# kirilllzaitsev/vision_mtl

Measured on AMD Instinct MI355X. Metric: images/sec fwd+bwd, basic model 128x256, higher is better.
Workload: dtype f32

## Files before the change

### include/vmtl.h

```cpp
#ifndef VMTL_H
#define VMTL_H

#ifdef __cplusplus
extern "C" {
#endif

#define VMTL_ACT_NONE 0
#define VMTL_ACT_RELU 1
#define VMTL_ACT_HSWISH 2
#define VMTL_ACT_HSIGMOID 3
#define VMTL_ACT_SIGMOID 4

#define VMTL_PREC_FP32 0
#define VMTL_PREC_BF16 1

const char* vmtl_version(void);
const char* vmtl_last_error_string(void);
int vmtl_reload_env(void);
int vmtl_timestamp(long long* out, void* stream);


int vmtl_conv2d_fwd(const float* x, const float* wp, const float* bias, float* y, float* stats,
                    int B, int H, int W, int Cs, int Ho, int Wo, int ldy, int Nw, int Cout,
                    int KH, int KW, int stride, int pad, int act, int shuffle, void* stream);
// ... 3 lines not shown
int vmtl_conv2d_ksplit(int B, int Ho, int Wo, int ldy, int Ktot);
int vmtl_conv2d_fwd_ws(const float* x, const float* wp, const float* bias, float* y, float* ws, int B, int H, int W, int Cs,
                       int Ho, int Wo, int ldy, int Nw, int Cout, int KH, int KW, int stride, int pad, void* stream);
int vmtl_conv2d_fwd_ws_p(const float* x, const float* wp, const float* bias, float* y, float* ws, int B, int H, int W,
                         int Cs, int Ho, int Wo, int ldy, int Nw, int Cout, int KH, int KW, int stride, int pad,
                         int precision, void* stream);
int vmtl_conv2d_stats_rows(int B, int Ho, int Wo, int ldy);
int vmtl_conv2d_stats_block(int B, int Ho, int Wo, int ldy);

int vmtl_conv1x1_stats_block(int M, int ldy, int Ks, int variant);
int vmtl_conv1x1_stats_rows(int M, int ldy, int Ks, int variant);
int vmtl_conv1x1_fwd(const float* x, const float* wp, const float* bias, float* y, float* stats, int M, int Ks, int ldy,
                     int Nw, int Cout, void* stream);
int vmtl_conv1x1_cat_fwd(const float* x, int K1, const float* x2, int K2s, const float* wp, const float* bias, float* y,
                         float* stats, int M, int ldy, int Nw, int Cout, void* stream);
int vmtl_conv1x1_cat_dgrad(const float* dy, const float* wp, float* dx, int N1, float* dx2, int N2s, int N2, int M,
                           int Ks, void* stream);
int vmtl_conv1x1_cat_wgrad(const float* x, int K1, const float* x2, int K2s, const float* dy, float* slabs, int splits,
                           int M, int ldy, int Nw, void* stream);
int vmtl_conv1x1_cat_wgrad_p(const float* x, int K1, const float* x2, int K2s, const float* dy, float* slabs, int splits,
                             int M, int ldy, int Nw, int precision, void* stream);
int vmtl_conv1x1_bn_fwd(const float* x, const float* coef_a, const float* coef_c, int act_in, float* a_out,
                        const float* wp, const float* bias, float* y, float* stats, int M, int Ks, int ldy, int Nw,
                        int Cout, void* stream);
int vmtl_conv1x1_bnbwd(const float* dy, const float* wp, float* dz, float* stats, const float* ez_x,
                       const float* ez_mean, const float* ez_invstd, const float* ez_gamma, const float* ez_beta,
                       int ez_act, int M, int Ks, int ldy, int Nw, int Cout, void* stream);
int vmtl_conv1x1_bn_res_fwd(const float* x, const float* coef_a, const float* coef_c, int act_in, const float* res,
                            float* a_out, const float* wp, const float* bias, float* y, float* stats, int M, int Ks,
                            int ldy, int Nw, int Cout, void* stream);
int vmtl_conv1x1_bnbwd_add(const float* dy, const float* wp, const float* addend, float* dz, float* stats,
                           const float* ez_x, const float* ez_mean, const float* ez_invstd, const float* ez_gamma,
                           const float* ez_beta, int ez_act, int M, int Ks, int ldy, int Nw, int Cout, void* stream);

int vmtl_conv2d_bnbwd(const float* x, const float* wp, float* y, float* stats, const float* ez_x, const float* ez_mean,
                      const float* ez_invstd, const float* ez_gamma, const float* ez_beta, int ez_act, int B, int H,
                      int W, int Cs, int Ho, int Wo, int ldy, int Nw, int Cout, int KH, int KW, int stride, int pad,
                      void* stream);
int vmtl_conv2d_bnbwd_p(const float* x, const float* wp, float* y, float* stats, const float* ez_x, const float* ez_mean,
                        const float* ez_invstd, const float* ez_gamma, const float* ez_beta, int ez_act, int B, int H,
                        int W, int Cs, int Ho, int Wo, int ldy, int Nw, int Cout, int KH, int KW, int stride, int pad,
                        int precision, void* stream);

int vmtl_conv2d_up2_fwd(const float* xl, const float* skip, const float* wp_eff, float* y, float* stats,
                        int B, int H2, int W2, int C0s, int C1s, int ldy, int Cout, void* stream);
int vmtl_conv2d_up2_fwd_p(const float* xl, const float* skip, const float* wp_eff, float* y, float* stats,
                          int B, int H2, int W2, int C0s, int C1s, int ldy, int Cout, int precision, void* stream);
int vmtl_conv2d_up2_stats_block(int B, int H2, int W2, int ldy);
int vmtl_conv2d_up2_ksplit(int B, int H2, int W2, int ldy, int Ktot);
int vmtl_conv2d_up2_fwd_ws(const float* xl, const float* skip, const float* wp_eff, float* y, float* ws, int B, int H2,
                           int W2, int C0s, int C1s, int ldy, int Cout, void* stream);
int vmtl_conv2d_up2_fwd_ws_p(const float* xl, const float* skip, const float* wp_eff, float* y, float* ws, int B, int H2,
                             int W2, int C0s, int C1s, int ldy, int Cout, int precision, void* stream);
int vmtl_pack_up2_fwd(const float* w, float* dst, int Cout, int C0, int C0s, int C1, int C1s, void* stream);
int vmtl_pack_up2_dgrad(const float* w, float* dst, int Cout, int Cos, int C0, int Cin, void* stream);
int vmtl_unpack_up2(const float* slabs, float* grad, int Cout, int Cos, int C0, int Cin, int nslabs, void* stream);

int vmtl_conv2d_wgrad_splits(int M, int Nw, int Ktot);
int vmtl_conv2d_wgrad(const float* x, const float* dy, float* slabs, int splits, int B, int H, int W, int Cs,
                      int Ho, int Wo, int ldy, int Nw, int KH, int KW, int stride, int pad, void* stream);
int vmtl_conv2d_wgrad_p(const float* x, const float* dy, float* slabs, int splits, int B, int H, int W, int Cs,
                        int Ho, int Wo, int ldy, int Nw, int KH, int KW, int stride, int pad, int precision,
                        void* stream);

int vmtl_conv3x3_wgrad_small_supported(int Cs, int ldy, int W);
int vmtl_conv3x3_wgrad_small_slabs(int B, int H, int W);
int vmtl_conv3x3_wgrad_small(const float* x, const float* dy, float* slabs, int nslabs, int B, int H, int W, int Cs,
                             int ldy, int Nw, void* stream);


int vmtl_conv3x3_small_supported(int Cs, int Nw);
int vmtl_conv3x3_small_tiles(int B, int H, int W);
int vmtl_conv3x3_small_stat_rows(int B, int H, int W);
int vmtl_conv3x3_small_stat_block(int B, int H, int W);
int vmtl_conv3x3_small(const float* x, const float* x2, const float* pa, const float* pb, const float* pc,
                       int act_in, float* a_out, const float* wp, const float* bias, float* y, float* yb, int Ca,
                       float* stats, int ep_mode, const float* ez_x, const float* ez_mean, const float* ez_invstd,
                       const float* ez_gamma, const float* ez_beta, int ez_act, int B, int H, int W, int Cs, int ldy,
                       int Nw, int Cout, void* stream);

int vmtl_dwconv_fwd(const float* x, const float* wp, float* y, int B, int H, int W, int Cs, int Ho, int Wo,
                    int K, int stride, int pad, void* stream);
int vmtl_dwconv_bn_stats_rows(int M, int Cs);
int vmtl_dwconv_bn_stats_block(int M, int Cs);
int vmtl_dwconv_bn_fwd(const float* x, const float* coef_a, const float* coef_c, int act, const float* wp, float* y,
                       float* a_out, float* partial, int B, int H, int W, int Cs, int Ho, int Wo, int K, int stride,
                       int pad, void* stream);
int vmtl_dwconv_bwd_data(const float* dy, const float* wp, float* dx, int B, int H, int W, int Cs, int Ho,
                         int Wo, int K, int stride, int pad, void* stream);
int vmtl_dwconv_bwd_data_add(const float* dy, const float* wp, const float* addend, float* dx, int B, int H, int W,
                             int Cs, int Ho, int Wo, int K, int stride, int pad, void* stream);
int vmtl_dwconv_bwd_weight_rows(int M, int Cs);
int vmtl_dwconv_bwd_weight(const float* x, const float* dy, float* partial, float* dw, int B, int H, int W,
                           int C, int Cs, int Ho, int Wo, int K, int stride, int pad, void* stream);

int vmtl_pack_weights(const float* src, float* dst, int R1, int R0, int T, int C, int Cs, long long sr1,
                      long long sr0, long long st, long long sc, int flip, void* stream);
int vmtl_pack_weights_scaled(const float* src, float* dst, int R1, int R0, int T, int C, int Cs, long long sr1,
                             long long sr0, long long st, long long sc, int flip, const float* scale, int sstride,
                             int smode, void* stream);
int vmtl_unpack_weights_stitch(const float* packed, float* grad, const float* w, const float* scale, int sstride,
                               float* ds, float* work, int R0, int T, int C, int Cs, int nslabs, long long slab_stride,
                               int reduce_all, void* stream);
int vmtl_pack_desc_bytes(void);
int vmtl_pack_weights_batch(const void* descs, int n, long long total, void* stream);
int vmtl_pack_weights_slice(const float* src, float* dst, int R0, int T, int C, int group, long long sr0,
// ... 113 lines not shown
```

### vision_mtl_amd/models/unet_mobilenetv3.py

```python
from __future__ import annotations

import math
import os
import typing as t

import torch
from torch import nn

from .. import layers as L
from ..ops import ACT_HSIGMOID, ACT_HSWISH, ACT_NONE, ACT_RELU

_ACT_CODE = {"relu": ACT_RELU, "hard_swish": ACT_HSWISH, None: ACT_NONE}


def _act_module(name):
    return {"relu": nn.ReLU, "hard_swish": nn.Hardswish, None: nn.Identity}[name]()


def make_divisible(v, divisor=8, min_value=None, round_limit=0.9):
    min_value = min_value or divisor
    new_v = max(min_value, int(v + divisor / 2) // divisor * divisor)
    if new_v < round_limit * v:
        new_v += divisor
    return new_v
# ... 227 lines not shown
            out = L.ops.conv2d(x.t, m.conv_stem.weight, None, L._pair(m.conv_stem.stride), L._pair(m.conv_stem.padding),
                               want_stats=train)
            raw0, st0 = out if train else (out, None)
            rpb0 = getattr(st0, "_vmtl_rpb", 0) if st0 is not None else 0
            y = first.run_pre(raw0, st0, rpb0, m.bn1, ACT_HSWISH)
        else:
            y = L.conv_bn_act(x, m.conv_stem, m.bn1, ACT_HSWISH)
        groups = [[0], [1], [2], [3, 4], [5, 6]]
        for g in groups[: self._depth]:
            for si in g:
                for blk in m.blocks[si]:
                    if fuse_stem and blk is first:
                        continue
                    y = blk.run(y)
            if g is groups[self._depth - 1]:
                feats.append(y.materialize() if isinstance(y, Pending) else y)
            elif isinstance(y, Pending):
                y.is_tap = True
                feats.append(y)
            else:
                y, tap = L.fork(y)
                feats.append(tap)
        return [f.act if isinstance(f, Pending) else f for f in feats]


class Conv2dReLU(nn.Sequential):
    def __init__(self, in_channels, out_channels):
        super().__init__(nn.Conv2d(in_channels, out_channels, 3, padding=1, bias=False), nn.BatchNorm2d(out_channels),
                         nn.ReLU(inplace=True))


class Attention(nn.Module):
    def __init__(self):
        super().__init__()
        self.attention = nn.Identity()


class DecoderBlock(nn.Module):

    def __init__(self, in_channels, skip_channels, out_channels):
        super().__init__()
        self.conv1 = Conv2dReLU(in_channels + skip_channels, out_channels)
        self.attention1 = Attention()
        self.conv2 = Conv2dReLU(out_channels, out_channels)
        self.attention2 = Attention()

    def run(self, x: L.Act, skip: t.Optional[L.Act]) -> L.Act:
        y = L.up2_conv_bn_act(x, skip, self.conv1[0], self.conv1[1], ACT_RELU)
        return L.conv_bn_act(y, self.conv2[0], self.conv2[1], ACT_RELU)

    def run_conv1_raw(self, x: L.Act, skip: t.Optional[L.Act]):
        c, bn = self.conv1[0], self.conv1[1]
        y, stats = L.ops.up2_conv(x.t, x.C, None if skip is None else skip.t, c.weight, want_stats=bn.training)
        rpb = 0
        if stats is not None:
            B, H2, W2, _ = x.t.shape
            rpb = L.ops.lib().raw("vmtl_conv2d_up2_stats_block")(B, H2, W2, y.shape[3])
        return L.Act(y, c.out_channels), stats, rpb


class UnetDecoder(nn.Module):
    def __init__(self, encoder_channels, decoder_channels):
        super().__init__()
        enc = list(encoder_channels[1:])[::-1]
        in_ch = [enc[0]] + list(decoder_channels[:-1])
        skip_ch = enc[1:] + [0]
        self.center = nn.Identity()
        self.blocks = nn.ModuleList([DecoderBlock(i, s, o) for i, s, o in zip(in_ch, skip_ch, decoder_channels)])
        for m in self.modules():
            if isinstance(m, nn.Conv2d):
                nn.init.kaiming_uniform_(m.weight, mode="fan_in", nonlinearity="relu")
            elif isinstance(m, nn.BatchNorm2d):
                nn.init.constant_(m.weight, 1)
                nn.init.constant_(m.bias, 0)

    def run(self, feats: t.List[L.Act], raw_tail: bool = False):
        feats = feats[1:][::-1]
        x, skips = feats[0], feats[1:]
        ops = L.ops
        raw = st = None
        rpb, bn, C = 0, None, 0
        for i, blk in enumerate(self.blocks):
            skip = skips[i] if i < len(skips) else None
            c1, bn1, c2, bn2 = blk.conv1[0], blk.conv1[1], blk.conv2[0], blk.conv2[1]
            skt = None if skip is None else skip.t
            if raw is None:
                raw, st, rpb = blk.run_conv1_raw(x, skip)
                raw = raw.t
            else:
                raw, st, rpb = ops.bn_act_conv(raw, st, rpb, bn, C, ACT_RELU, c1.weight, skip=skt, up2=True,
                                               want_stats=bn1.training)
            bn, C = bn1, c1.out_channels
            if raw_tail and i == len(self.blocks) - 1:
                return L.Act(raw, C), st, rpb
            raw, st, rpb = ops.bn_act_conv(raw, st, rpb, bn, C, ACT_RELU, c2.weight, want_stats=bn2.training)
            bn, C = bn2, c2.out_channels
        return L.bn_act(L.Act(raw, C), bn, ACT_RELU, stats=st, stats_rpb=rpb)


class Activation(nn.Module):
    def __init__(self, name=None):
        super().__init__()
        if name not in (None, "identity"):
            raise NotImplementedError("only activation=None is used by the reference (basic_model.py:13)")
        self.activation = nn.Identity()


class SegmentationHead(nn.Sequential):

    def __init__(self, in_channels, out_channels, kernel_size=3, activation=None, upsampling=1):
# ... 51 lines not shown
```

### vision_mtl_amd/ops.py

```python
from __future__ import annotations

import contextlib
import os
import weakref

import torch

from ._lib import lib
from .precision import conv_prec_code

ACT_NONE, ACT_RELU, ACT_HSWISH, ACT_HSIGMOID, ACT_SIGMOID = 0, 1, 2, 3, 4
ACT_CODES = {None: 0, "none": 0, "relu": 1, "hardswish": 2, "hardsigmoid": 3, "sigmoid": 4}


def ceil4(c: int) -> int:
    return (c + 3) // 4 * 4


def _stream() -> int:
    return torch.cuda.current_stream().cuda_stream


def _req(t: torch.Tensor, name: str = "tensor") -> torch.Tensor:
    if not t.is_cuda:
# ... 325 lines not shown


def _wgrad(x, dy, B, H, W, Cs, Ho, Wo, ldy, Nw, KH, KW, stride, pad, flop, xflop=None, prec=0):
    if (KH == 3 and KW == 3 and stride == 1 and pad == 1 and B * H * W * max(Cs, ldy) * 4 < 1 << 32
            and lib().raw("vmtl_conv3x3_wgrad_small_supported")(Cs, ldy, W)):
        ns = lib().raw("vmtl_conv3x3_wgrad_small_slabs")(B, H, W)
        slabs = _empty((ns, Nw, 9 * Cs), x)
        _k("vmtl_conv3x3_wgrad_small", _flop=flop, _xflop=xflop, x=x, dy=dy, slabs=slabs, nslabs=ns, B=B, H=H, W=W, Cs=Cs, ldy=ldy,
           Nw=Nw)
        return slabs, ns
    splits = lib().raw("vmtl_conv2d_wgrad_splits")(B * Ho * Wo, Nw, KH * KW * Cs)
    slabs = _empty((splits, Nw, KH * KW * Cs), x)
    _kp("vmtl_conv2d_wgrad", prec, _flop=flop, _xflop=xflop, x=x, dy=dy, slabs=slabs, splits=splits, B=B, H=H, W=W, Cs=Cs, Ho=Ho, Wo=Wo,
       ldy=ldy, Nw=Nw, KH=KH, KW=KW, stride=stride, pad=pad)
    return slabs, splits


def _colsum(a, b, M, C, Cs, mode=0, reduce_all=0, out=None):
    partial = _empty((_reduce_rows(M) + 1, Cs), a)
    if out is None:
        out = _empty((1 if reduce_all else C,), a)
    _k("vmtl_colsum", a=a, b=b, M=M, C=C, Cs=Cs, mode=mode, reduce_all=reduce_all, partial=partial, out=out)
    return out


def _bias_grad(bias, slot, dy, M, Cout, ldy, zero, fork):
    arena = getattr(bias, "_vmtl_arena", None) if slot is not None else None
    if zero:
        if slot is None:
            db = _empty((Cout,), dy)
            _k("vmtl_fill_zero", p=db, n=Cout)
            return db
        capturing = torch.cuda.is_current_stream_capturing()
        if arena is None or id(bias) not in arena._zero_bias or (capturing and side.enabled and not side.task_mode):
            with side.branch(True, M, fork, dy):
                _k("vmtl_fill_zero", p=slot, n=Cout)
            if arena is not None and not capturing:
                arena._zero_bias.add(id(bias))
        return None
    with side.branch(slot is not None, M, fork, dy):
        db = _colsum(dy, None, M, Cout, ldy, out=slot)
    if slot is not None:
        if arena is not None:
            arena._zero_bias.discard(id(bias))
        return None
    return db


FUSE_DW = os.environ.get("VMTL_FUSE_DW", "1") != "0"
_PW = os.environ.get("VMTL_PW", "1") != "0"
_PW_MAX_ROWS = int(os.environ.get("VMTL_PW_MAX_ROWS", str(1 << 21)))


def _is_pw(B, Ho, Wo, KH, KW, stride, pad, shuffle=0):
    return _PW and KH == 1 and KW == 1 and stride == 1 and pad == 0 and not shuffle and B * Ho * Wo <= _PW_MAX_ROWS


_SMALL_MIN_ROWS = int(os.environ.get("VMTL_SMALL_MIN_ROWS", str(1 << 16)))


def conv_ksplit(B, Ho, Wo, Cs, ldy, KH, KW, stride, pad, shuffle=0) -> int:
    if shuffle or _is_pw(B, Ho, Wo, KH, KW, stride, pad, shuffle):
        return 1
    return lib().raw("vmtl_conv2d_ksplit")(B, Ho, Wo, ldy, KH * KW * Cs)


_SMALL_STATS = os.environ.get("VMTL_SMALL_STATS", "1") != "0"


def _small_route(B, H, W, Cs, ldy, KH, KW, stride, pad, shuffle=0, with_stats=False) -> bool:
    if shuffle or KH != 3 or KW != 3 or stride != 1 or pad != 1 or ldy > 36 or B * H * W < _SMALL_MIN_ROWS:
        return False
    if B * H * W * 36 > 0x7FFFFFFF:
        return False
    if not conv3x3_small_supported(Cs, ldy):
        return False
    return not with_stats or (_SMALL_STATS and H % 4 == 0 and W % 32 == 0)


def conv_stats_geometry(B, Ho, Wo, Cs, ldy, KH, KW, stride, pad):
    if _small_route(B, Ho, Wo, Cs, ldy, KH, KW, stride, pad, with_stats=True):
        return lib().raw("vmtl_conv3x3_small_stat_rows")(B, Ho, Wo), lib().raw("vmtl_conv3x3_small_stat_block")(B, Ho, Wo)
    if _is_pw(B, Ho, Wo, KH, KW, stride, pad):
        M = B * Ho * Wo
        return lib().raw("vmtl_conv1x1_stats_rows")(M, ldy, Cs, 0), lib().raw("vmtl_conv1x1_stats_block")(M, ldy, Cs, 0)
    return lib().raw("vmtl_conv2d_stats_rows")(B, Ho, Wo, ldy), lib().raw("vmtl_conv2d_stats_block")(B, Ho, Wo, ldy)


def _conv_launch(x, wp, bias, y, stats, B, H, W, Cs, Ho, Wo, ldy, Nw, Cout, KH, KW, stride, pad, shuffle=0, cin=None,
                 algo_flop=None, prec=0):
    flop = 2.0 * B * Ho * Wo * Nw * KH * KW * (Cs if cin is None else cin)
    if _is_pw(B, Ho, Wo, KH, KW, stride, pad, shuffle):
        _k("vmtl_conv1x1_fwd", _flop=flop if algo_flop is None else algo_flop, _xflop=flop, x=x, wp=wp, bias=bias, y=y,
           stats=stats, M=B * Ho * Wo, Ks=Cs, ldy=ldy, Nw=Nw, Cout=Cout)
        return
    if _small_route(B, H, W, Cs, ldy, KH, KW, stride, pad, shuffle, with_stats=stats is not None):
        _small(x, wp, y, B, H, W, Cs, ldy, Nw, Cout, flop if algo_flop is None else algo_flop, bias=bias, stats=stats,
               ep_mode=1 if stats is not None else 0)
        return
    if stats is None and not shuffle:
        ks = lib().raw("vmtl_conv2d_ksplit")(B, Ho, Wo, ldy, KH * KW * Cs)
        if ks > 1:
            ws = _empty((ks, B * Ho * Wo, ldy), x)
            _kp("vmtl_conv2d_fwd_ws", prec, _flop=flop if algo_flop is None else algo_flop, _xflop=flop, x=x, wp=wp, bias=bias, y=y,
               ws=ws, B=B, H=H, W=W, Cs=Cs, Ho=Ho, Wo=Wo, ldy=ldy, Nw=Nw, Cout=Cout, KH=KH, KW=KW, stride=stride, pad=pad)
            return
# ... 272 lines not shown
                Ks = Ca + Cbs
                ns = lib().raw("vmtl_conv2d_wgrad_splits")(M, Cout, Ks)
                slabs = _empty((ns, Cout, Ks), xa)
                _kp("vmtl_conv1x1_cat_wgrad", ctx.prec, _flop=2.0 * M * Cout * Cin, x=xa, K1=Ca, x2=xb, K2s=Cbs, dy=dy, slabs=slabs,
                   splits=ns, M=M, ldy=ldy, Nw=Cout)
                unpack(slabs, None, 1, Cout, 1, Cin, Ks, 0, Cin, 1, 1, out=flat, nslabs=ns)
            dw = None if sw is not None else dwt
        if has_bias and ctx.needs_input_grad[3]:
            db = _bias_grad(ctx.bias, sbias, dy, M, Cout, ldy, zero_bias, fork)
        return dxa, dxb, dw, db, None, None, None


def conv1x1_cat_supported(xa, Ca, xb):
    return _PW and Ca % 4 == 0 and xa.shape[3] == Ca and xa.shape[0] * xa.shape[1] * xa.shape[2] <= _PW_MAX_ROWS \
        and tuple(xa.shape[:3]) == tuple(xb.shape[:3]) and os.environ.get("VMTL_CAT_CONV", "1") != "0"


def conv1x1_cat(xa, xb, Cb, weight, bias=None, want_stats=False, zero_bias_grad=False):
    y, stats = _Conv1x1Cat.apply(xa, xb, weight, bias, Cb, want_stats, zero_bias_grad)
    if stats is not None:
        stats._vmtl_rpb = lib().raw("vmtl_conv1x1_stats_block")(y.shape[0] * y.shape[1] * y.shape[2], y.shape[3],
                                                                xa.shape[3] + xb.shape[3], 0)
    return y, stats


class _Up2Conv(torch.autograd.Function):

    @staticmethod
    def forward(ctx, xl, skip, weight, C0, want_stats):
        xl, weight = _req(xl, "xl"), _req(weight, "weight")
        B, H2, W2, C0s = xl.shape
        Cout, Cin = weight.shape[0], weight.shape[1]
        if tuple(weight.shape[2:]) != (3, 3):
            raise ValueError("up2_conv: 3x3 kernels only")
        if skip is not None:
            skip = _req(skip, "skip")
            C1s = skip.shape[3]
            if tuple(skip.shape[:3]) != (B, 2 * H2, 2 * W2):
                raise ValueError("up2_conv: skip must be at twice the resolution of xl")
        else:
            C1s = 0
        C1 = Cin - C0
        if ceil4(C0) != C0s or ceil4(C1) != C1s or (C1 > 0) != (skip is not None):
            raise ValueError(f"up2_conv: weight has {Cin} input channels, sources hold {C0s}+{C1s} storage channels")
        ldy = ceil4(Cout)
        Ktot = 4 * C0s + 9 * C1s
        wp = packs.get_custom(weight, "up2_fwd", (4, Cout, Ktot), lambda w, dst: _k(
            "vmtl_pack_up2_fwd", w=w, dst=dst, Cout=Cout, C0=C0, C0s=C0s, C1=C1, C1s=C1s))
        y = _empty((B, 2 * H2, 2 * W2, ldy), xl)
        stats = None
        M = B * 4 * H2 * W2
        prec = ctx.prec = conv_prec_code()
        ks = lib().raw("vmtl_conv2d_up2_ksplit")(B, H2, W2, ldy, Ktot)
        if ks > 1:
            _kp("vmtl_conv2d_up2_fwd_ws", prec, _flop=2.0 * M * Cout * 9 * Cin, _xflop=2.0 * M * Cout * (4 * C0 + 9 * C1), xl=xl,
               skip=skip, wp_eff=wp, y=y, ws=_empty((ks, B, 2 * H2, 2 * W2, ldy), xl), B=B, H2=H2, W2=W2, C0s=C0s, C1s=C1s,
               ldy=ldy, Cout=Cout)
        else:
            if want_stats:
                bm = lib().raw("vmtl_conv2d_up2_stats_block")(B, H2, W2, ldy)
                Mq = B * H2 * W2
                if Mq % bm == 0:
                    stats = _empty((4 * (Mq // bm), 2, ldy), xl)
            _kp("vmtl_conv2d_up2_fwd", prec, _flop=2.0 * M * Cout * 9 * Cin, _xflop=2.0 * M * Cout * (4 * C0 + 9 * C1), xl=xl,
               skip=skip, wp_eff=wp, y=y, stats=stats, B=B, H2=H2, W2=W2, C0s=C0s, C1s=C1s, ldy=ldy, Cout=Cout)
        ctx.save_for_backward(xl, skip, weight)
        ctx.cfg = (C0, C1, stats.shape[0] if stats is not None else 0)
        ctx.slot = _slot(weight)
        ctx.set_materialize_grads(False)
        if stats is not None:
            ctx.mark_non_differentiable(stats)
        return y, stats

    @staticmethod
    def backward(ctx, dy, _dstats):
        xl, skip, weight = ctx.saved_tensors
        C0, C1, _ = ctx.cfg
        if dy is None:
            return None, None, None, None
        dy = _req(dy, "dy")
        B, H2, W2, C0s = xl.shape
        Cout, Cin = weight.shape[0], weight.shape[1]
        H, W, ldy = 2 * H2, 2 * W2, dy.shape[3]
        dxl = dskip = dw = None
        stamp(f"main up2 M={B * H * W} N={Cout} Cin={Cin}")
        fork = side.mark()
        if ctx.needs_input_grad[0]:
            wd = packs.get_custom(weight, "up2_dgrad", (C0, 16 * ldy), lambda w, dst: _k(
                "vmtl_pack_up2_dgrad", w=w, dst=dst, Cout=Cout, Cos=ldy, C0=C0, Cin=Cin))
            dxl = _empty((B, H2, W2, C0s), xl)
            _conv_launch(dy, wd, None, dxl, None, B, H, W, ldy, H2, W2, C0s, C0, C0, 4, 4, 2, 1, cin=Cout,
                         algo_flop=2.0 * B * H * W * C0 * 9 * Cout, prec=ctx.prec)
        if skip is not None and ctx.needs_input_grad[1]:
            C1s = skip.shape[3]
            wds = packs.get(weight, "up2_dskip", (1, C1, 9, Cout, ldy, 0, 9, 1, Cin * 9, 1), offset=C0 * 9)
            dskip = _empty((B, H, W, C1s), xl)
            _conv_launch(dy, wds, None, dskip, None, B, H, W, ldy, H, W, C1s, C1, C1, 3, 3, 1, 1, cin=Cout, prec=ctx.prec)
        if ctx.needs_input_grad[2]:
            dw = _empty(weight.shape, xl) if ctx.slot is None else ctx.slot
            with side.branch(ctx.slot is not None, B * H * W, fork, dy, xl, skip):
                slabs, ns = _wgrad(dy, xl, B, H, W, ldy, H2, W2, C0s, C0, 4, 4, 2, 1, 2.0 * B * H * W * Cout * 9 * C0,
                                   xflop=2.0 * B * H2 * W2 * C0 * 16 * Cout, prec=ctx.prec)
                _k("vmtl_unpack_up2", slabs=slabs, grad=dw, Cout=Cout, Cos=ldy, C0=C0, Cin=Cin, nslabs=ns)
                if skip is not None:
                    C1s = skip.shape[3]
                    slabs, ns = _wgrad(skip, dy, B, H, W, C1s, H, W, ldy, Cout, 3, 3, 1, 1,
                                       2.0 * B * H * W * Cout * 9 * C1, prec=ctx.prec)
# ... 6 lines not shown

class _BNActConv(torch.autograd.Function):

    @staticmethod
    def forward(ctx, x, stats, rpb, gamma, beta, rm, rv, nbt, weight, skip, cfg):
        C, training, momentum, eps, act, up2, want_stats = cfg
        x, weight = _req(x, "x"), _req(weight, "weight")
        B, H, W, Cs = x.shape
        M = B * H * W
        Cout, Cin = weight.shape[0], weight.shape[1]
        if ceil4(C) != Cs or tuple(weight.shape[2:]) != (3, 3):
            raise ValueError("bn_act_conv: 3x3 weight over x's channels expected")
        mean, invstd = _empty((Cs,), x), _empty((Cs,), x)
        a = _empty(x.shape, x)
        if training:
            if stats is not None:
                partial, nblk = stats, stats.shape[0]
            else:
                partial, nblk, rpb = _empty((_reduce_rows(M), 2, Cs), x), 0, 0
            if 0 < nblk <= _BN_FUSE_ROWS:
                _k("vmtl_bn_apply_fused", x=x, partial=partial, nblk=nblk, rows_per_blk=rpb, eps=eps, momentum=momentum,
                   running_mean=rm, running_var=rv, num_batches_tracked=nbt, save_mean=mean, save_invstd=invstd,
                   gamma=gamma, beta=beta, mul=None, res=None, y=a, M=M, C=C, Cs=Cs, act=act)
            else:
                _k("vmtl_bn_stats", x=x, M=M, C=C, Cs=Cs, partial=partial, nblk_from_conv=nblk, rows_per_blk_from_conv=rpb,
                   eps=eps, momentum=momentum, running_mean=rm, running_var=rv, num_batches_tracked=nbt, save_mean=mean,
                   save_invstd=invstd)
                _k("vmtl_bn_apply", x=x, mean=mean, invstd=invstd, gamma=gamma, beta=beta, mul=None, res=None, y=a, M=M,
                   C=C, Cs=Cs, act=act)
        else:
            _k("vmtl_bn_eval_stats", running_mean=rm, running_var=rv, C=C, Cs=Cs, eps=eps, save_mean=mean, save_invstd=invstd)
            _k("vmtl_bn_apply", x=x, mean=mean, invstd=invstd, gamma=gamma, beta=beta, mul=None, res=None, y=a, M=M, C=C,
               Cs=Cs, act=act)
        prec = ctx.prec = conv_prec_code()
        ldy = ceil4(Cout)
        ostats, orpb = None, 0
        if up2:
            if skip is not None:
                skip = _req(skip, "skip")
                C1s = skip.shape[3]
                if tuple(skip.shape[:3]) != (B, 2 * H, 2 * W):
                    raise ValueError("bn_act_conv(up2): skip must be at twice the resolution of x")
            else:
                C1s = 0
            C1 = Cin - C
            if ceil4(C1) != C1s or (C1 > 0) != (skip is not None):
                raise ValueError("bn_act_conv(up2): weight channels do not match x + skip")
            Ktot = 4 * Cs + 9 * C1s
            wp = packs.get_custom(weight, "up2_fwd", (4, Cout, Ktot), lambda w, dst: _k(
                "vmtl_pack_up2_fwd", w=w, dst=dst, Cout=Cout, C0=C, C0s=Cs, C1=C1, C1s=C1s))
            y = _empty((B, 2 * H, 2 * W, ldy), x)
            Mo = 4 * M
            ks = lib().raw("vmtl_conv2d_up2_ksplit")(B, H, W, ldy, Ktot)
            if ks > 1:
                _kp("vmtl_conv2d_up2_fwd_ws", prec, _flop=2.0 * Mo * Cout * 9 * Cin, _xflop=2.0 * Mo * Cout * (4 * C + 9 * C1),
                   xl=a, skip=skip, wp_eff=wp, y=y, ws=_empty((ks, B, 2 * H, 2 * W, ldy), x), B=B, H2=H, W2=W, C0s=Cs,
                   C1s=C1s, ldy=ldy, Cout=Cout)
            else:
                if want_stats:
                    bm = lib().raw("vmtl_conv2d_up2_stats_block")(B, H, W, ldy)
                    if M % bm == 0:
                        ostats, orpb = _empty((4 * (M // bm), 2, ldy), x), bm
                _kp("vmtl_conv2d_up2_fwd", prec, _flop=2.0 * Mo * Cout * 9 * Cin, _xflop=2.0 * Mo * Cout * (4 * C + 9 * C1), xl=a,
                   skip=skip, wp_eff=wp, y=y, stats=ostats, B=B, H2=H, W2=W, C0s=Cs, C1s=C1s, ldy=ldy, Cout=Cout)
        else:
            if Cin != C or skip is not None:
                raise ValueError("bn_act_conv: weight expects x's channels (skip only with up2)")
            wp = packs.get(weight, "fwd", (1, Cout, 9, Cin, Cs, 0, Cin * 9, 1, 9, 0))
            y = _empty((B, H, W, ldy), x)
            if want_stats and conv_ksplit(B, H, W, Cs, ldy, 3, 3, 1, 1) == 1:
                rows, orpb = conv_stats_geometry(B, H, W, Cs, ldy, 3, 3, 1, 1)
                ostats = _empty((rows, 2, ldy), x)
            _conv_launch(a, wp, None, y, ostats, B, H, W, Cs, H, W, ldy, Cout, Cout, 3, 3, 1, 1, cin=Cin, prec=prec)
        ctx.save_for_backward(x, a, skip, weight, mean, invstd, gamma, beta)
        ctx.cfg = (C, training, act, up2)
        ctx.slots = (_slot(gamma), _slot(beta), _slot(weight))
        ctx.orpb = orpb
        ctx.set_materialize_grads(False)
        if ostats is not None:
            ctx.mark_non_differentiable(ostats)
        return y, ostats

    @staticmethod
    def backward(ctx, dy, _dstats):
        x, a, skip, weight, mean, invstd, gamma, beta = ctx.saved_tensors
        C, training, act, up2 = ctx.cfg
        sg, sb, sw = ctx.slots
        if dy is None:
            return (None,) * 11
        dy = _req(dy, "dy")
        B, H, W, Cs = x.shape
        M = B * H * W
        Cout, Cin = weight.shape[0], weight.shape[1]
        ldy = dy.shape[3]
        stamp(f"main bnconv M={dy.shape[0] * dy.shape[1] * dy.shape[2]} N={Cout} Cin={Cin}")
        fork = side.mark()
        if up2:
            Hd, Wd = 2 * H, 2 * W
            wd = packs.get_custom(weight, "up2_dgrad", (C, 16 * ldy), lambda w, dst: _k(
                "vmtl_pack_up2_dgrad", w=w, dst=dst, Cout=Cout, Cos=ldy, C0=C, Cin=Cin))
            geo = dict(B=B, H=Hd, W=Wd, Cs=ldy, Ho=H, Wo=W, ldy=Cs, Nw=C, Cout=C, KH=4, KW=4, stride=2, pad=1)
            flop, xflop = 2.0 * B * Hd * Wd * C * 9 * Cout, 2.0 * M * C * 16 * Cout
        else:
            Hd, Wd = H, W
            wd = packs.get(weight, "dgrad", (1, Cin, 9, Cout, ldy, 0, 9, 1, Cin * 9, 1))
            geo = dict(B=B, H=H, W=W, Cs=ldy, Ho=H, Wo=W, ldy=Cs, Nw=Cin, Cout=Cin, KH=3, KW=3, stride=1, pad=1)
            flop = xflop = 2.0 * M * Cin * 9 * Cout
# ... 13 lines not shown
                rows = lib().raw("vmtl_conv2d_stats_rows")(B, H, W, Cs)
                part = _empty((rows, 2, Cs), x)
                _kp("vmtl_conv2d_bnbwd", ctx.prec, _flop=flop, _xflop=xflop, x=dy, wp=wd, y=dz, stats=part, ez_x=x, ez_mean=mean,
                   ez_invstd=invstd, ez_gamma=gamma, ez_beta=beta, ez_act=act, **geo)
            _k("vmtl_bn_bwd_finalize", partial=part, nblk=rows, M=M, C=C, Cs=Cs, sum_dz=dbeta, sum_dzx=dgamma, mean=None,
               invstd=None, gamma=None, training=1 if training else 0, coef_a=None, coef_b=None, coef_c=None)
            if dx is not None:
                _k("vmtl_bn_bwd_apply", x=x, dz=dz, mean=mean, invstd=invstd, gamma=gamma, sum_dz=dbeta, sum_dzx=dgamma,
                   dx=dx, M=M, C=C, Cs=Cs, training=1 if training else 0)
        else:
            da = _empty(x.shape, x)
            _conv_launch(dy, wd, None, da, None, geo["B"], geo["H"], geo["W"], geo["Cs"], geo["Ho"], geo["Wo"], geo["ldy"],
                         geo["Nw"], geo["Cout"], geo["KH"], geo["KW"], geo["stride"], geo["pad"], cin=Cout, algo_flop=flop,
                         prec=ctx.prec)
            part = _empty((_reduce_rows(M), 2, Cs), x)
            _k("vmtl_bn_bwd", x=x, dy=da, mean=mean, invstd=invstd, gamma=gamma, beta=beta, mul=None, dmul=None,
               partial=part, sum_dz=dbeta, sum_dzx=dgamma, dx=dx if dx is not None else _empty(x.shape, x), M=M, C=C, Cs=Cs,
               act=act, training=1 if training else 0)
        dskip = None
        if up2 and skip is not None and ctx.needs_input_grad[9]:
            C1, C1s = Cin - C, skip.shape[3]
            wds = packs.get(weight, "up2_dskip", (1, C1, 9, Cout, ldy, 0, 9, 1, Cin * 9, 1), offset=C * 9)
            dskip = _empty(skip.shape, x)
            _conv_launch(dy, wds, None, dskip, None, B, Hd, Wd, ldy, Hd, Wd, C1s, C1, C1, 3, 3, 1, 1, cin=Cout, prec=ctx.prec)
        dw = _empty(weight.shape, x) if sw is None else sw
        with side.branch(sw is not None, B * Hd * Wd, fork, dy, a, skip):
            if up2:
                slabs, ns = _wgrad(dy, a, B, Hd, Wd, ldy, H, W, Cs, C, 4, 4, 2, 1, 2.0 * B * Hd * Wd * Cout * 9 * C,
                                   xflop=2.0 * M * C * 16 * Cout, prec=ctx.prec)
                _k("vmtl_unpack_up2", slabs=slabs, grad=dw, Cout=Cout, Cos=ldy, C0=C, Cin=Cin, nslabs=ns)
                if skip is not None:
                    C1, C1s = Cin - C, skip.shape[3]
                    slabs, ns = _wgrad(skip, dy, B, Hd, Wd, C1s, Hd, Wd, ldy, Cout, 3, 3, 1, 1,
                                       2.0 * B * Hd * Wd * Cout * 9 * C1, prec=ctx.prec)
                    unpack(slabs, None, 1, Cout, 9, C1, C1s, 0, Cin * 9, 1, 9, out=dw.view(-1)[C * 9:], nslabs=ns)
            else:
                slabs, ns = _wgrad(a, dy, B, H, W, Cs, H, W, ldy, Cout, 3, 3, 1, 1, 2.0 * M * Cout * 9 * Cin, prec=ctx.prec)
                unpack(slabs, weight.shape, 1, Cout, 9, Cin, Cs, 0, Cin * 9, 1, 9, out=dw, nslabs=ns)
            stamp(f"side bnconv N={Cout} Cin={Cin}")
        nif = lambda g, slot: None if slot is not None else g
        return dx, None, None, nif(dgamma, sg), nif(dbeta, sb), None, None, None, nif(dw, sw), dskip, None


def bn_act_conv(x, stats, rpb, bn, C, act, weight, skip=None, up2=False, want_stats=True):
    if bn.momentum is None:
        raise NotImplementedError("BatchNorm2d(momentum=None) (cumulative moving average) is not implemented")
    cfg = (C, bn.training, float(bn.momentum), bn.eps, act, bool(up2), bool(want_stats))
    y, ostats = _BNActConv.apply(x, stats, rpb, bn.weight, bn.bias, bn.running_mean, bn.running_var,
                                 bn.num_batches_tracked, weight, skip, cfg)
    orpb = 0
    if ostats is not None:
        B, H, W, _ = x.shape
        ldy = y.shape[3]
        orpb = (lib().raw("vmtl_conv2d_up2_stats_block")(B, H, W, ldy) if up2
                else conv_stats_geometry(B, H, W, x.shape[3], ldy, 3, 3, 1, 1)[1])
    return y, ostats, orpb


def up2_conv(xl, C0, skip, weight, want_stats=False):
    y, stats = _Up2Conv.apply(xl, skip, weight, C0, want_stats)
    if stats is not None:
        stats._vmtl_rpb = lib().raw("vmtl_conv2d_up2_stats_block")(xl.shape[0], xl.shape[1], xl.shape[2], y.shape[3])
    return y, stats


def conv2d(x, weight, bias=None, stride=1, pad=0, want_stats=False, zero_bias_grad=False, stitch=None):
    y, stats = _Conv2d.apply(x, weight, bias, stride, pad, want_stats, zero_bias_grad,
                             None if stitch is None else stitch[0], 0 if stitch is None else int(stitch[1]))
    if stats is not None:
        stats._vmtl_rpb = conv_stats_geometry(y.shape[0], y.shape[1], y.shape[2], x.shape[3], y.shape[3], weight.shape[2],
                                              weight.shape[3], stride, pad)[1]
    return (y, stats) if want_stats else y


class _ConvT2x2(torch.autograd.Function):

    @staticmethod
    def forward(ctx, x, weight, bias):
        x = _req(x, "x")
        weight = _req(weight, "weight")
        B, H, W, Cs = x.shape
        Cin, Cout = weight.shape[0], weight.shape[1]
        if tuple(weight.shape[2:]) != (2, 2) or ceil4(Cin) != Cs:
            raise ValueError("conv_transpose2x2: weight must be (Cin, Cout, 2, 2) matching the input channels")
        ldy = ceil4(Cout)
        wp = packs.get(weight, "ct_fwd", (4, Cout, 1, Cin, Cs, 1, 4, 0, Cout * 4, 0))
        y = _empty((B, 2 * H, 2 * W, ldy), x)
        _conv_launch(x, wp, bias, y, None, B, H, W, Cs, H, W, ldy, 4 * Cout, Cout, 1, 1, 1, 0, shuffle=1, cin=Cin)
        ctx.save_for_backward(x, weight)
        ctx.has_bias = bias is not None
        ctx.slots = (_slot(weight), _slot(bias))
        return y

    @staticmethod
    def backward(ctx, dy):
        x, weight = ctx.saved_tensors
        dy = _req(dy, "dy")
        B, H, W, Cs = x.shape
        Cin, Cout = weight.shape[0], weight.shape[1]
        ldy = dy.shape[3]
        dx = dw = db = None
        fork = side.mark()
        if ctx.needs_input_grad[0]:
            wd = packs.get(weight, "ct_bwd", (1, Cin, 4, Cout, ldy, 0, Cout * 4, 1, 4, 0))
            dx = _empty((B, H, W, Cs), x)
            _conv_launch(dy, wd, None, dx, None, B, 2 * H, 2 * W, ldy, H, W, Cs, Cin, Cin, 2, 2, 2, 0, cin=Cout)
        if ctx.needs_input_grad[1]:
            with side.branch(ctx.slots[0] is not None, B * H * W, fork, x, dy):
                slabs, ns = _wgrad(dy, x, B, 2 * H, 2 * W, ldy, H, W, Cs, Cin, 2, 2, 2, 0,
                                   2.0 * B * H * W * Cin * 4 * Cout)
                dw = unpack(slabs, weight.shape, 1, Cin, 4, Cout, ldy, 0, Cout * 4, 1, 4, out=ctx.slots[0], nslabs=ns)
            if ctx.slots[0] is not None:
                dw = None
        if ctx.has_bias and ctx.needs_input_grad[2]:
            with side.branch(ctx.slots[1] is not None, B * 4 * H * W, fork, dy):
# ... 1069 lines not shown
```

Measured before the change: 2557.

## Add halo-tiled fused upsample+concat+conv3x3 kernel for two decoder shapes

Adds a specialized HIP kernel that stages a low-resolution input halo and a skip-connection halo in LDS once per tile. It then computes the upsample-by-2 3x3 convolution with fp32 MFMA from those staged tiles, with a scalar tail for leftover output channels. The kernel writes the output through an LDS transpose and emits per-tile BN mean and M2 statistics. It is routed only for two hardcoded channel configurations with fp32 precision and no k-split, replacing the generic up2 kernel there. This aims to reduce redundant global reads of the input, at the cost of more LDS use and a new statistics-block geometry that callers must query.

After: 2599 (median of 6 runs). 1.02x the previous value.

```diff
diff --git a/include/vmtl.h b/include/vmtl.h
--- a/include/vmtl.h
+++ b/include/vmtl.h
@@ -79,6 +79,11 @@
                            int W2, int C0s, int C1s, int ldy, int Cout, void* stream);
 int vmtl_conv2d_up2_fwd_ws_p(const float* xl, const float* skip, const float* wp_eff, float* y, float* ws, int B, int H2,
                              int W2, int C0s, int C1s, int ldy, int Cout, int precision, void* stream);
+int vmtl_conv2d_up2_halo(const float* xl, const float* skip, const float* wp_eff, float* y, float* stats,
+                         int B, int H2, int W2, int C0s, int C1s, int ldy, int Cout, void* stream);
+int vmtl_conv2d_up2_halo_supported(int B, int H2, int W2, int C0s, int C1s, int ldy, int Cout);
+int vmtl_conv2d_up2_halo_stat_rows(int B, int H2, int W2, int C0s, int C1s, int ldy, int Cout);
+int vmtl_conv2d_up2_halo_stat_block(int C0s, int C1s, int ldy, int Cout);
 int vmtl_pack_up2_fwd(const float* w, float* dst, int Cout, int C0, int C0s, int C1, int C1s, void* stream);
 int vmtl_pack_up2_dgrad(const float* w, float* dst, int Cout, int Cos, int C0, int Cin, void* stream);
 int vmtl_unpack_up2(const float* slabs, float* grad, int Cout, int Cos, int C0, int Cin, int nslabs, void* stream);
diff --git a/vision_mtl_amd/csrc/conv_up2_halo.hip b/vision_mtl_amd/csrc/conv_up2_halo.hip
--- /dev/null
+++ b/vision_mtl_amd/csrc/conv_up2_halo.hip
@@ -0,0 +1,342 @@
+#include "common.h"
+
+#define UH_TW 16
+
+struct Up2HaloP {
+  const float* xl;
+  const float* skip;
+  const float* wp;
+  float* y;
+  float* stats;
+  int B, H2, W2, Nw;
+  int tiles_x, tiles_y;
+  int xl_bytes, skip_bytes, wp_bytes;
+};
+
+template <int C0S, int C1S, int TM, int TN, int NT>
+struct UhCfg {
+  static constexpr int SP0 = C0S / 4, SP1 = C1S / 4;
+  static constexpr int FG0 = SP0 / 4, RS0 = SP0 % 4, NGF0 = 4 * FG0, NR0 = 4 * RS0, NGR0 = (NR0 + 3) / 4;
+  static constexpr int FG1 = SP1 / 4, NGF1 = 9 * FG1;
+  static constexpr int NG = NGF0 + NGR0 + NGF1;
+  static constexpr int KQ = 4 * SP0 + 9 * SP1;
+  static constexpr int HX0 = UH_TW + 2, HX1 = 2 * UH_TW + 2;
+  static constexpr int NP0 = ((TM + 2) * HX0) | 1;
+  static constexpr int NP1 = SP1 > 0 ? ((2 * TM + 2) * HX1) | 1 : 0;
+  static constexpr int NST0 = (TM + 2) * HX0 * SP0, NST1 = (2 * TM + 2) * HX1 * SP1;
+  static constexpr int IT0 = (NST0 + 255) / 256, IT1 = (NST1 + 255) / 256;
+  static constexpr int NROWS = 16 * TN;
+  static constexpr int OS = NROWS + 4;
+  static constexpr int SQ = OS / 4;
+  static constexpr int NPX = 2 * TM * 2 * UH_TW;
+  static constexpr int ZQ = SP0 * NP0 + SP1 * NP1;
+  static constexpr int HALO4 = ZQ + 1;
+  static constexpr int OT4 = NPX * SQ;
+  static constexpr int MAIN4 = HALO4 > OT4 ? HALO4 : OT4;
+  static constexpr int RED4 = 256 + 32;
+  static constexpr int LDS_BYTES = (MAIN4 + RED4) * 16;
+  static_assert(C1S % 16 == 0, "skip channels: whole k-groups per tap");
+  static_assert(NT >= 1 && NT <= 4, "tail columns");
+  static_assert(256 / SQ * SQ <= 256, "statistics lanes");
+};
+
+__device__ __forceinline__ f32x4 uh_bload(__amdgpu_buffer_rsrc_t r, unsigned off) {
+  return __builtin_bit_cast(f32x4, __builtin_amdgcn_raw_buffer_load_b128(r, off, 0, 0));
+}
+
+template <int C0S, int C1S, int TM, int TN, int NT>
+__global__ __launch_bounds__(256) __attribute__((amdgpu_waves_per_eu(2))) void conv_up2_halo_kernel(Up2HaloP p) {
+  using C = UhCfg<C0S, C1S, TM, TN, NT>;
+  constexpr int SP0 = C::SP0, SP1 = C::SP1, FG0 = C::FG0, RS0 = C::RS0, NGF0 = C::NGF0, NR0 = C::NR0, NGR0 = C::NGR0;
+  constexpr int FG1 = C::FG1, NG = C::NG, KQ = C::KQ, HX0 = C::HX0, HX1 = C::HX1, NP0 = C::NP0, NP1 = C::NP1;
+  constexpr int NROWS = C::NROWS, OS = C::OS, SQ = C::SQ, NPX = C::NPX, ZQ = C::ZQ;
+  constexpr int NB = TN + NT;
+  constexpr unsigned OOB = 0xFFFFFFFFu;
+
+  extern __shared__ __attribute__((aligned(16))) f32x4 smem4[];
+  f32x4* halo = smem4;
+  float* otile = reinterpret_cast<float*>(smem4);
+  f32x4* red = smem4 + C::MAIN4;
+
+  const int tid = threadIdx.x;
+  const int lane = tid & 63, wv = tid >> 6;
+  const int l15 = lane & 15, lq = lane >> 4;
+  const int pa = wv >> 1, pb = wv & 1;
+
+  int t = blockIdx.x;
+  const int tx = t % p.tiles_x;
+  t /= p.tiles_x;
+  const int ty = t % p.tiles_y, b = t / p.tiles_y;
+  const int hl0 = ty * TM, wl0 = tx * UH_TW;
+  const int H = 2 * p.H2, W = 2 * p.W2;
+
+  const __amdgpu_buffer_rsrc_t rs_x = __builtin_amdgcn_make_buffer_rsrc((void*)p.xl, 0, p.xl_bytes, 0x00020000);
+  const __amdgpu_buffer_rsrc_t rs_s =
+      __builtin_amdgcn_make_buffer_rsrc((void*)(C1S > 0 ? p.skip : p.xl), 0, C1S > 0 ? p.skip_bytes : 0, 0x00020000);
+  const __amdgpu_buffer_rsrc_t rs_w = __builtin_amdgcn_make_buffer_rsrc((void*)p.wp, 0, p.wp_bytes, 0x00020000);
+
+  unsigned wrow[NB];
+#pragma unroll
+  for (int j = 0; j < NB; ++j) {
+    const int n = j < TN ? 16 * j + l15 : NROWS + (j - TN);
+    wrow[j] = n < p.Nw ? (unsigned)((wv * p.Nw + n) * KQ) * 16u : 0x80000000u;
+  }
+  int arem[NGR0 > 0 ? NGR0 : 1];
+  unsigned krem[NGR0 > 0 ? NGR0 : 1];
+#pragma unroll
+  for (int h = 0; h < NGR0; ++h) {
+    const int r = 4 * h + lq;
+    if (r < NR0) {
+      const int tap = r / (RS0 > 0 ? RS0 : 1), s = FG0 * 4 + r % (RS0 > 0 ? RS0 : 1);
+      arem[h] = s * NP0 + (pa + (tap >> 1)) * HX0 + pb + (tap & 1) + l15;
+      krem[h] = (unsigned)(tap * SP0 + s) * 16u;
+    } else {
+      arem[h] = -1;
+      krem[h] = 0x40000000u;
+    }
+  }
+  const int a0 = lq * NP0 + pa * HX0 + pb + l15;
+  const int a1 = SP0 * NP0 + lq * NP1 + pa * HX1 + pb + 2 * l15;
+
+  {
+    f32x4 r0[C::IT0], r1[C::IT1 > 0 ? C::IT1 : 1];
+#pragma unroll
+    for (int it = 0; it < C::IT0; ++it) {
+      const int f = tid + 256 * it;
+      const int pp = f / SP0, s = f - pp * SP0;
+      const int hy = pp / HX0, hx = pp - hy * HX0;
+      const int gh = hl0 - 1 + hy, gw = wl0 - 1 + hx;
+      const bool ok = f < C::NST0 && (unsigned)gh < (unsigned)p.H2 && (unsigned)gw < (unsigned)p.W2;
+      r0[it] = uh_bload(rs_x, ok ? (unsigned)((b * p.H2 + gh) * p.W2 + gw) * (unsigned)(C0S * 4) + 16u * s : OOB);
+    }
+#pragma unroll
+    for (int it = 0; it < C::IT1; ++it) {
+      const int f = tid + 256 * it;
+      const int pp = f / (SP1 > 0 ? SP1 : 1), s = f - pp * SP1;
+      const int hy = pp / HX1, hx = pp - hy * HX1;
+      const int gh = 2 * hl0 - 1 + hy, gw = 2 * wl0 - 1 + hx;
+      const bool ok = f < C::NST1 && (unsigned)gh < (unsigned)H && (unsigned)gw < (unsigned)W;
+      r1[it] = uh_bload(rs_s, ok ? (unsigned)((b * H + gh) * W + gw) * (unsigned)(C1S * 4) + 16u * s : OOB);
+    }
+#pragma unroll
+    for (int it = 0; it < C::IT0; ++it) {
+      const int f = tid + 256 * it;
+      const int pp = f / SP0, s = f - pp * SP0;
+      if (f < C::NST0) halo[s * NP0 + pp] = r0[it];
+    }
+#pragma unroll
+    for (int it = 0; it < C::IT1; ++it) {
+      const int f = tid + 256 * it;
+      const int pp = f / (SP1 > 0 ? SP1 : 1), s = f - pp * SP1;
+      if (f < C::NST1) halo[SP0 * NP0 + s * NP1 + pp] = r1[it];
+    }
+    if (tid == 0) halo[ZQ] = (f32x4){0.f, 0.f, 0.f, 0.f};
+  }
+  __syncthreads();
+
+  f32x4 acc[TM][TN];
+  f32x2 tacc[TM][NT];
+#pragma unroll
+  for (int i = 0; i < TM; ++i) {
+#pragma unroll
+    for (int j = 0; j < TN; ++j) acc[i][j] = (f32x4){0.f, 0.f, 0.f, 0.f};
+#pragma unroll
+    for (int tt = 0; tt < NT; ++tt) tacc[i][tt] = (f32x2){0.f, 0.f};
+  }
+  auto group = [&](int g, unsigned& koff, int& ai, int& istep) {
+    if (g < NGF0) {
+      const int tap = g / FG0, cb = (g % FG0) * 4;
+      koff = (unsigned)(tap * SP0 + cb + lq) * 16u;
+      ai = a0 + cb * NP0 + (tap >> 1) * HX0 + (tap & 1);
+      istep = HX0;
+    } else if (g < NGF0 + NGR0) {
+      koff = krem[g - NGF0];
+      ai = arem[g - NGF0];
+      istep = HX0;
+    } else {
+      const int g1 = g - NGF0 - NGR0;
+      const int tap = g1 / (FG1 > 0 ? FG1 : 1), cb = (g1 % (FG1 > 0 ? FG1 : 1)) * 4;
+      koff = (unsigned)(4 * SP0 + tap * SP1 + cb + lq) * 16u;
+      ai = a1 + cb * NP1 + (tap / 3) * HX1 + tap % 3;
+      istep = 2 * HX1;
+    }
+  };
+  auto load_b = [&](int g, f32x4 (&bq)[NB]) {
+    unsigned koff;
+    int ai, istep;
+    group(g, koff, ai, istep);
+#pragma unroll
+    for (int j = 0; j < NB; ++j) bq[j] = uh_bload(rs_w, wrow[j] + koff);
+  };
+  auto load_a = [&](int g, f32x4 (&aq)[TM]) {
+    unsigned koff;
+    int ai, istep;
+    group(g, koff, ai, istep);
+#pragma unroll
+    for (int i = 0; i < TM; ++i) aq[i] = halo[ai < 0 ? ZQ : ai + i * istep];
+  };
+  auto mma = [&](const f32x4 (&aq)[TM], const f32x4 (&bq)[NB]) {
+#pragma unroll
+    for (int e = 0; e < 4; ++e)
+#pragma unroll
+      for (int i = 0; i < TM; ++i)
+#pragma unroll
+        for (int j = 0; j < TN; ++j) acc[i][j] = __builtin_amdgcn_mfma_f32_16x16x4f32(aq[i][e], bq[j][e], acc[i][j], 0, 0, 0);
+#pragma unroll
+    for (int tt = 0; tt < NT; ++tt) {
+      const f32x4 w = bq[TN + tt];
+      const f32x2 lo = __builtin_shufflevector(w, w, 0, 1), hi = __builtin_shufflevector(w, w, 2, 3);
+#pragma unroll
+      for (int i = 0; i < TM; ++i) {
+        tacc[i][tt] += __builtin_shufflevector(aq[i], aq[i], 0, 1) * lo;
+        tacc[i][tt] += __builtin_shufflevector(aq[i], aq[i], 2, 3) * hi;
+        asm volatile("" : "+v"(tacc[i][tt]));
+      }
+    }
+  };
+  f32x4 bq[3][NB], aq[2][TM];
+  load_b(0, bq[0]);
+  if (NG > 1) load_b(1, bq[1]);
+  load_a(0, aq[0]);
+#pragma unroll
+  for (int g = 0; g < NG; ++g) {
+    if (g + 2 < NG) load_b(g + 2, bq[(g + 2) % 3]);
+    if (g + 1 < NG) load_a(g + 1, aq[(g + 1) & 1]);
+    mma(aq[g & 1], bq[g % 3]);
+    if (g + 2 < NG) __builtin_amdgcn_sched_group_barrier(0x020, NB, 0);
+    if (g + 1 < NG) __builtin_amdgcn_sched_group_barrier(0x100, TM, 0);
+    __builtin_amdgcn_sched_group_barrier(0x008, 4 * TM * TN, 0);
+    __builtin_amdgcn_sched_group_barrier(0x002, 4 * TM * NT + 8, 0);
+    __builtin_amdgcn_sched_barrier(0);
+  }
+
+  float tv[TM][NT];
+#pragma unroll
+  for (int tt = 0; tt < NT; ++tt)
+#pragma unroll
+    for (int i = 0; i < TM; ++i) {
+      float v = tacc[i][tt][0] + tacc[i][tt][1];
+      v += __shfl_xor(v, 16, 64);
+      v += __shfl_xor(v, 32, 64);
+      tv[i][tt] = v;
+    }
+  __syncthreads();
+#pragma unroll
+  for (int i = 0; i < TM; ++i) {
+    const int prow = (2 * i + pa) * (2 * UH_TW) + pb;
+#pragma unroll
+    for (int j = 0; j < TN; ++j)
+#pragma unroll
+      for (int r = 0; r < 4; ++r) otile[(prow + 2 * (4 * lq + r)) * OS + 16 * j + l15] = acc[i][j][r];
+    if (lq == 0) {
+#pragma unroll
+      for (int tt = 0; tt < 4; ++tt) otile[(prow + 2 * l15) * OS + NROWS + tt] = tt < NT ? tv[i][tt < NT ? tt : 0] : 0.f;
+    }
+  }
+  __syncthreads();
+
+  const f32x4* ot4 = reinterpret_cast<const f32x4*>(otile);
+  constexpr int SIT = (NPX * SQ + 255) / 256;
+#pragma unroll
+  for (int it = 0; it < SIT; ++it) {
+    const int f = tid + 256 * it;
+    if (f < NPX * SQ) {
+      const int px = f / SQ, q = f - px * SQ;
+      const int gy = 2 * hl0 + px / (2 * UH_TW), gx = 2 * wl0 + px % (2 * UH_TW);
+      if (gy < H && gx < W)
+        *reinterpret_cast<f32x4*>(p.y + ((unsigned)((b * H + gy) * W + gx) * (unsigned)OS + 4u * q)) = ot4[f];
+    }
+  }
+
+  if (p.stats != nullptr) {
+    constexpr int G = 256 / SQ;
+    const int q = tid % SQ, gi = tid / SQ;
+    f32x4 s = {0.f, 0.f, 0.f, 0.f};
+    if (gi < G)
+      for (int px = gi; px < NPX; px += G) s += ot4[px * SQ + q];
+    red[tid] = s;
+    __syncthreads();
+    if (tid < SQ) {
+      f32x4 m = {0.f, 0.f, 0.f, 0.f};
+      for (int k = 0; k < G; ++k) m += red[k * SQ + tid];
+      red[256 + tid] = m * (1.f / (float)NPX);
+    }
+    __syncthreads();
+    const f32x4 m = red[256 + q];
+    f32x4 c = {0.f, 0.f, 0.f, 0.f};
+    if (gi < G)
+      for (int px = gi; px < NPX; px += G) {
+        const f32x4 d = ot4[px * SQ + q] - m;
+        c += d * d;
+      }
+    red[tid] = c;
+    __syncthreads();
+    if (tid < SQ) {
+      f32x4 m2 = {0.f, 0.f, 0.f, 0.f};
+      for (int k = 0; k < G; ++k) m2 += red[k * SQ + tid];
+      *reinterpret_cast<f32x4*>(p.stats + ((size_t)blockIdx.x * 2 + 0) * OS + 4 * tid) = m;
+      *reinterpret_cast<f32x4*>(p.stats + ((size_t)blockIdx.x * 2 + 1) * OS + 4 * tid) = m2;
+    }
+  }
+}
+
+template <int C0S, int C1S, int TM, int TN, int NT>
+static int launch_up2_halo(Up2HaloP& p, hipStream_t st) {
+  using C = UhCfg<C0S, C1S, TM, TN, NT>;
+  static_assert(C::LDS_BYTES <= 64 * 1024, "at least two workgroups per CU");
+  if (hipFuncSetAttribute(reinterpret_cast<const void*>(&conv_up2_halo_kernel<C0S, C1S, TM, TN, NT>),
+                          hipFuncAttributeMaxDynamicSharedMemorySize, C::LDS_BYTES) != hipSuccess)
+    return VMTL_ERR_LAUNCH;
+  p.tiles_x = cdiv(p.W2, UH_TW);
+  p.tiles_y = cdiv(p.H2, TM);
+  hipLaunchKernelGGL((conv_up2_halo_kernel<C0S, C1S, TM, TN, NT>), dim3(p.B * p.tiles_x * p.tiles_y), dim3(256),
+                     C::LDS_BYTES, st, p);
+  return vmtl_check_launch();
+}
+
+static int up2_halo_tm(int C0s, int C1s, int ldy, int Cout) {
+  if (C0s == 68 && C1s == 0 && Cout == 33 && ldy == 36) return 4;
+  if (C0s == 136 && C1s == 16 && Cout == 67 && ldy == 68) return 2;
+  return 0;
+}
+
+static bool up2_halo_fits(int B, int H2, int W2, int C0s, int C1s, int ldy) {
+  const long long px = (long long)B * H2 * W2;
+  return px * C0s * 4 <= 0x7fffffffLL && 4 * px * C1s * 4 <= 0x7fffffffLL && 4 * px * ldy * 4 <= 0x7fffffffLL;
+}
+
+extern "C" int vmtl_conv2d_up2_halo_supported(int B, int H2, int W2, int C0s, int C1s, int ldy, int Cout) {
+  return B > 0 && H2 > 0 && W2 > 0 && up2_halo_tm(C0s, C1s, ldy, Cout) > 0 && up2_halo_fits(B, H2, W2, C0s, C1s, ldy);
+}
+
+extern "C" int vmtl_conv2d_up2_halo_stat_block(int C0s, int C1s, int ldy, int Cout) {
+  return 4 * UH_TW * up2_halo_tm(C0s, C1s, ldy, Cout);
+}
+
+extern "C" int vmtl_conv2d_up2_halo_stat_rows(int B, int H2, int W2, int C0s, int C1s, int ldy, int Cout) {
+  const int tm = up2_halo_tm(C0s, C1s, ldy, Cout);
+  if (tm == 0 || B <= 0 || H2 <= 0 || W2 <= 0 || H2 % tm || W2 % UH_TW) return 0;
+  return B * (H2 / tm) * (W2 / UH_TW);
+}
+
+extern "C" int vmtl_conv2d_up2_halo(const float* xl, const float* skip, const float* wp_eff, float* y, float* stats,
+                                    int B, int H2, int W2, int C0s, int C1s, int ldy, int Cout, void* stream) {
+  VMTL_ENTER();
+  if (!xl || !wp_eff || !y || B <= 0 || H2 <= 0 || W2 <= 0 || C0s <= 0 || C1s < 0 || Cout <= 0 || Cout > ldy)
+    return VMTL_ERR_ARG;
+  if ((skip == nullptr) != (C1s == 0)) return VMTL_ERR_ARG;
+  const int tm = up2_halo_tm(C0s, C1s, ldy, Cout);
+  if (tm == 0) return VMTL_ERR_UNSUPPORTED;
+  if (stats != nullptr && vmtl_conv2d_up2_halo_stat_rows(B, H2, W2, C0s, C1s, ldy, Cout) == 0) return VMTL_ERR_ARG;
+  if (!up2_halo_fits(B, H2, W2, C0s, C1s, ldy)) return VMTL_ERR_UNSUPPORTED;
+  const long long px = (long long)B * H2 * W2;
+  Up2HaloP p;
+  p.xl = xl; p.skip = skip; p.wp = wp_eff; p.y = y; p.stats = stats;
+  p.B = B; p.H2 = H2; p.W2 = W2; p.Nw = Cout;
+  p.xl_bytes = (int)(px * C0s * 4);
+  p.skip_bytes = (int)(4 * px * C1s * 4);
+  p.wp_bytes = 4 * Cout * (4 * C0s + 9 * C1s) * 4;
+  hipStream_t st = (hipStream_t)stream;
+  if (tm == 4) return launch_up2_halo<68, 0, 4, 2, 1>(p, st);
+  return launch_up2_halo<136, 16, 2, 4, 3>(p, st);
+}
diff --git a/vision_mtl_amd/models/unet_mobilenetv3.py b/vision_mtl_amd/models/unet_mobilenetv3.py
--- a/vision_mtl_amd/models/unet_mobilenetv3.py
+++ b/vision_mtl_amd/models/unet_mobilenetv3.py
@@ -303,10 +303,7 @@
     def run_conv1_raw(self, x: L.Act, skip: t.Optional[L.Act]):
         c, bn = self.conv1[0], self.conv1[1]
         y, stats = L.ops.up2_conv(x.t, x.C, None if skip is None else skip.t, c.weight, want_stats=bn.training)
-        rpb = 0
-        if stats is not None:
-            B, H2, W2, _ = x.t.shape
-            rpb = L.ops.lib().raw("vmtl_conv2d_up2_stats_block")(B, H2, W2, y.shape[3])
+        rpb = 0 if stats is None else stats._vmtl_rpb
         return L.Act(y, c.out_channels), stats, rpb
 
 
diff --git a/vision_mtl_amd/ops.py b/vision_mtl_amd/ops.py
--- a/vision_mtl_amd/ops.py
+++ b/vision_mtl_amd/ops.py
@@ -401,6 +401,26 @@
 _PW_MAX_ROWS = int(os.environ.get("VMTL_PW_MAX_ROWS", str(1 << 21)))
 
 
+_UP2_HALO = os.environ.get("VMTL_UP2_HALO", "1") != "0"
+
+
+def _up2_halo_route(B, H2, W2, C0s, C1s, ldy, Cout, prec) -> bool:
+    return (_UP2_HALO and prec == 0 and bool(lib().raw("vmtl_conv2d_up2_halo_supported")(B, H2, W2, C0s, C1s, ldy, Cout))
+            and lib().raw("vmtl_conv2d_up2_ksplit")(B, H2, W2, ldy, 4 * C0s + 9 * C1s) == 1)
+
+
+def up2_stats_geometry(B, H2, W2, C0s, C1s, ldy, Cout, prec=None):
+    prec = conv_prec_code() if prec is None else prec
+    if _up2_halo_route(B, H2, W2, C0s, C1s, ldy, Cout, prec):
+        return (lib().raw("vmtl_conv2d_up2_halo_stat_rows")(B, H2, W2, C0s, C1s, ldy, Cout),
+                lib().raw("vmtl_conv2d_up2_halo_stat_block")(C0s, C1s, ldy, Cout))
+    if lib().raw("vmtl_conv2d_up2_ksplit")(B, H2, W2, ldy, 4 * C0s + 9 * C1s) > 1:
+        return 0, 0
+    bm = lib().raw("vmtl_conv2d_up2_stats_block")(B, H2, W2, ldy)
+    Mq = B * H2 * W2
+    return (4 * (Mq // bm), bm) if Mq % bm == 0 else (0, bm)
+
+
 def _is_pw(B, Ho, Wo, KH, KW, stride, pad, shuffle=0):
     return _PW and KH == 1 and KW == 1 and stride == 1 and pad == 0 and not shuffle and B * Ho * Wo <= _PW_MAX_ROWS
 
@@ -779,7 +799,14 @@
         M = B * 4 * H2 * W2
         prec = ctx.prec = conv_prec_code()
         ks = lib().raw("vmtl_conv2d_up2_ksplit")(B, H2, W2, ldy, Ktot)
-        if ks > 1:
+        if _up2_halo_route(B, H2, W2, C0s, C1s, ldy, Cout, prec):
+            if want_stats:
+                rows, _ = up2_stats_geometry(B, H2, W2, C0s, C1s, ldy, Cout, prec)
+                if rows:
+                    stats = _empty((rows, 2, ldy), xl)
+            _k("vmtl_conv2d_up2_halo", _flop=2.0 * M * Cout * 9 * Cin, _xflop=2.0 * M * Cout * (4 * C0 + 9 * C1), xl=xl,
+               skip=skip, wp_eff=wp, y=y, stats=stats, B=B, H2=H2, W2=W2, C0s=C0s, C1s=C1s, ldy=ldy, Cout=Cout)
+        elif ks > 1:
             _kp("vmtl_conv2d_up2_fwd_ws", prec, _flop=2.0 * M * Cout * 9 * Cin, _xflop=2.0 * M * Cout * (4 * C0 + 9 * C1), xl=xl,
                skip=skip, wp_eff=wp, y=y, ws=_empty((ks, B, 2 * H2, 2 * W2, ldy), xl), B=B, H2=H2, W2=W2, C0s=C0s, C1s=C1s,
                ldy=ldy, Cout=Cout)
@@ -892,7 +919,14 @@
             y = _empty((B, 2 * H, 2 * W, ldy), x)
             Mo = 4 * M
             ks = lib().raw("vmtl_conv2d_up2_ksplit")(B, H, W, ldy, Ktot)
-            if ks > 1:
+            if _up2_halo_route(B, H, W, Cs, C1s, ldy, Cout, prec):
+                if want_stats:
+                    rows, bm = up2_stats_geometry(B, H, W, Cs, C1s, ldy, Cout, prec)
+                    if rows:
+                        ostats, orpb = _empty((rows, 2, ldy), x), bm
+                _k("vmtl_conv2d_up2_halo", _flop=2.0 * Mo * Cout * 9 * Cin, _xflop=2.0 * Mo * Cout * (4 * C + 9 * C1), xl=a,
+                   skip=skip, wp_eff=wp, y=y, stats=ostats, B=B, H2=H, W2=W, C0s=Cs, C1s=C1s, ldy=ldy, Cout=Cout)
+            elif ks > 1:
                 _kp("vmtl_conv2d_up2_fwd_ws", prec, _flop=2.0 * Mo * Cout * 9 * Cin, _xflop=2.0 * Mo * Cout * (4 * C + 9 * C1),
                    xl=a, skip=skip, wp_eff=wp, y=y, ws=_empty((ks, B, 2 * H, 2 * W, ldy), x), B=B, H2=H, W2=W, C0s=Cs,
                    C1s=C1s, ldy=ldy, Cout=Cout)
@@ -1012,7 +1046,7 @@
     if ostats is not None:
         B, H, W, _ = x.shape
         ldy = y.shape[3]
-        orpb = (lib().raw("vmtl_conv2d_up2_stats_block")(B, H, W, ldy) if up2
+        orpb = (up2_stats_geometry(B, H, W, x.shape[3], 0 if skip is None else skip.shape[3], ldy, weight.shape[0])[1] if up2
                 else conv_stats_geometry(B, H, W, x.shape[3], ldy, 3, 3, 1, 1)[1])
     return y, ostats, orpb
 
@@ -1020,7 +1054,8 @@
 def up2_conv(xl, C0, skip, weight, want_stats=False):
     y, stats = _Up2Conv.apply(xl, skip, weight, C0, want_stats)
     if stats is not None:
-        stats._vmtl_rpb = lib().raw("vmtl_conv2d_up2_stats_block")(xl.shape[0], xl.shape[1], xl.shape[2], y.shape[3])
+        stats._vmtl_rpb = up2_stats_geometry(xl.shape[0], xl.shape[1], xl.shape[2], xl.shape[3],
+                                             0 if skip is None else skip.shape[3], y.shape[3], weight.shape[0])[1]
     return y, stats
 
 
```
